# mlvlab/RPO

Hardware: AMD Instinct MI355X
Metric: images/sec (train step, ViT-B/16 K=24) (higher is better)
Workload: dtype bf16

## Files before the change

### rpo_amd/csrc/gemm_ws.hip

```cpp
#include "common.h"

#include <type_traits>

namespace {

struct WsParams {
  const char* A; int64_t lda;
  const char* Wp;
  char* C; int64_t ldc;
  int M, N, K;
  int tiles_m, tiles_n, split_k; int64_t split_stride;
  const float* bias;
  const float* resid; int64_t ldr;
  char* aux; int64_t ldaux; int aux_row0; int aux_mode;
  char* out2; int64_t ldout2; float* stats_out;
  const float* stats_in; const float* ln_colsum; float ln_eps; int ln_group;
  const char* pf_ptr; int64_t pf_bytes;
};

template <int N> __device__ __forceinline__ void ws_wait_vmcnt() {
  asm volatile("s_waitcnt vmcnt(%0)" ::"n"(N) : "memory");
}

__device__ __forceinline__ void ws_lds_barrier() { asm volatile("s_waitcnt lgkmcnt(0)\n\ts_barrier" ::: "memory"); }

template <int MT_, int NT_>
struct WsCfg {
  static constexpr int MT = MT_, NT = NT_, SLOTS = 2, THREADS = 256;
  static constexpr int BM = MT * 32, BN = NT * 32;
  static constexpr int SLOT_BYTES = BM * 128;
  static constexpr int WAVE_RING = SLOTS * SLOT_BYTES;
  static constexpr int RING_BYTES = 4 * WAVE_RING;
  static constexpr int FROW = BN * 4 + 16;
  static constexpr int PART_BYTES = 32 * FROW;
  static constexpr int STAGE_BYTES = 2 * 4 * PART_BYTES;
  static constexpr int STATS_BYTES = BM * 8;
  static constexpr int SMEM = (RING_BYTES > STAGE_BYTES ? RING_BYTES : STAGE_BYTES) + STATS_BYTES;
  static constexpr int DA = MT * 4;
  static constexpr int DW = NT * 4;
};

__device__ __forceinline__ float ws_row8_sum(float v) {
  v += __int_as_float(__builtin_amdgcn_update_dpp(0, __float_as_int(v), 0xB1, 0xf, 0xf, false));
  v += __int_as_float(__builtin_amdgcn_update_dpp(0, __float_as_int(v), 0x4E, 0xf, 0xf, false));
  v += __int_as_float(__builtin_amdgcn_update_dpp(0, __float_as_int(v), 0x141, 0xf, 0xf, false));
  return v;
}

__device__ __forceinline__ float2 ws_ln_finish(float mu_sum, float m2_sum, float sq_sum, int G, int K, float eps) {
  const float mu = mu_sum / (float)G;
  const float between = fmaxf(fmaf(-(float)G * mu, mu, sq_sum), 0.f);
  const float m2 = fmaf((float)(K / G), between, m2_sum);
  return make_float2(mu, rsqrtf(m2 / (float)K + eps));
}

template <typename T, typename TOut, int EPI, typename CF>
__global__ __launch_bounds__(256, 1) void gemm_ws_kernel(const WsParams p) {
  extern __shared__ __attribute__((aligned(128))) char smem[];
  constexpr int MT = CF::MT, NT = CF::NT;
  typedef const __attribute__((address_space(1))) void* gptr_t;
  typedef __attribute__((address_space(3))) void* lptr_t;
  const int tid = threadIdx.x;
  const int lane = tid & 63;
  const int wave = __builtin_amdgcn_readfirstlane(tid >> 6);
  const int half = lane >> 5, l31 = lane & 31;
  RPO_STAMP(0); RPO_STAMP_RT(62);

  int tile_m, tile_n, ksl;
  {
    const int nwg = gridDim.x, bid = blockIdx.x;
    const int qd = nwg >> 3, rm = nwg & 7, xcd = bid & 7;
    const int wg = (xcd < rm ? xcd * (qd + 1) : rm * (qd + 1) + (xcd - rm) * qd) + (bid >> 3);
    tile_m = wg % p.tiles_m;
    const int rest = wg / p.tiles_m;
    tile_n = rest % p.tiles_n;
    ksl = rest / p.tiles_n;
  }
  const int m0 = tile_m * CF::BM, n0 = tile_n * CF::BN;
  const int nch_all = p.K >> 6;
  const int wc0 = (int)(((int64_t)nch_all * ksl) / p.split_k), wc1 = (int)(((int64_t)nch_all * (ksl + 1)) / p.split_k);
  const int nwc = wc1 - wc0;
  const int c_lo = wc0 + (nwc * wave) / 4, c_hi = wc0 + (nwc * (wave + 1)) / 4;
  const int nc = c_hi - c_lo;

  uint32_t aoff[CF::DA];
  const int arow = lane >> 3;
  const uint32_t apark = (uint32_t)(arow * 128 + (((lane & 7) ^ ((arow >> 1) & 7)) << 4));
#pragma unroll
  for (int j = 0; j < CF::DA; ++j)
    aoff[j] = (uint32_t)min(m0 + 8 * j + arow, p.M - 1) * (uint32_t)(p.lda * 2) + (lane & 7) * 16;
  char* const ring = smem + wave * CF::WAVE_RING;
  const int KS = p.K >> 4;
  const char* wb[NT];
#pragma unroll
  for (int tn = 0; tn < NT; ++tn) {
    const int nb = min(n0 / 32 + tn, p.N / 32 - 1);
    wb[tn] = p.Wp + ((int64_t)nb * KS * 64 + lane) * 16;
  }
  const int sw = (l31 >> 1) & 7;
  uint32_t frag_off[4];
#pragma unroll
  for (int s = 0; s < 4; ++s) frag_off[s] = l31 * 128 + (((2 * s + half) ^ sw) << 4);

  f32x16_t acc[NT][MT];
#pragma unroll
  for (int a = 0; a < NT; ++a)
#pragma unroll
    for (int b = 0; b < MT; ++b)
#pragma unroll
      for (int r = 0; r < 16; ++r) acc[a][b][r] = 0.0f;

  constexpr bool IS_LN = EPI == RPO_EPI_LN_BIAS || EPI == RPO_EPI_LN_BIAS_QGELU;
  constexpr bool IS_QG = EPI == RPO_EPI_BIAS_QGELU || EPI == RPO_EPI_LN_BIAS_QGELU;
  constexpr bool HAS_BIAS = EPI == RPO_EPI_BIAS || EPI == RPO_EPI_BIAS_QGELU || EPI == RPO_EPI_BIAS_RESID || IS_LN;
  float2* const row_stats = reinterpret_cast<float2*>(smem + CF::SMEM - CF::STATS_BYTES);
  float2 lnp[IS_LN ? 16 : 1];
  const int G = IS_LN ? p.K / p.ln_group : 1;
  if constexpr (IS_LN) {
    if (tid < CF::BM) {
      const float2* ps = reinterpret_cast<const float2*>(p.stats_in) + (int64_t)min(m0 + tid, p.M - 1) * G;
#pragma unroll
      for (int g = 0; g < 16; ++g) lnp[g] = ps[min(g, G - 1)];
    }
  }
  const int row8 = lane >> 3, c8 = lane & 7;
  constexpr bool PRE_F32 = EPI == RPO_EPI_BIAS_RESID;
  constexpr bool PRE_AUX = EPI == RPO_EPI_QGELU_BWD;
  typedef __attribute__((ext_vector_type(4))) uint32_t u32x4_t;
  typedef __attribute__((ext_vector_type(2))) uint32_t u32x2_t;
  u32x4_t pre[(PRE_F32 || PRE_AUX) ? MT : 1][(PRE_F32 || PRE_AUX) ? NT : 1];
  if constexpr (PRE_F32 || PRE_AUX) {
    const bool wide = PRE_F32 || !p.aux_mode;
    const char* base = PRE_F32 ? reinterpret_cast<const char*>(p.resid) : p.aux;
    const int64_t ld = PRE_F32 ? p.ldr : p.ldaux;
#pragma unroll
    for (int tm = 0; tm < MT; ++tm) {
      const int m = min(m0 + tm * 32 + 8 * wave + row8, p.M - 1);
#pragma unroll
      for (int j = 0; j < NT; ++j) {
        const int n = min(n0 + 32 * j + 4 * c8, p.N - 4);
        if (wide) {
          pre[tm][j] = *reinterpret_cast<const u32x4_t*>(base + ((int64_t)m * ld + n) * 4);
        } else {
          const u32x2_t u = *reinterpret_cast<const u32x2_t*>(base + ((int64_t)m * ld + n) * 2);
          pre[tm][j] = u32x4_t{u.x, u.y, 0u, 0u};
        }
      }
    }
  }
  float4 b4[NT], s4[NT];
#pragma unroll
  for (int j = 0; j < NT; ++j) {
    const int n = min(n0 + 32 * j + 4 * c8, p.N - 4);
    b4[j] = HAS_BIAS ? *reinterpret_cast<const float4*>(p.bias + n) : make_float4(0.f, 0.f, 0.f, 0.f);
    s4[j] = IS_LN ? *reinterpret_cast<const float4*>(p.ln_colsum + n) : make_float4(0.f, 0.f, 0.f, 0.f);
  }
  bf16x8_t areg[CF::DA];
  bf16x8_t w[NT][4];
  constexpr int PPS = CF::DA / 4;
#define WS_PROLOGUE(NEXT)                                                                                              \
  {                                                                                                                      \
    const char* src = p.A + (int64_t)c_lo * 128;                                                                         \
    _Pragma("unroll") for (int j = 0; j < CF::DA; ++j) areg[j] = *reinterpret_cast<const bf16x8_t*>(src + aoff[j]);      \
    _Pragma("unroll") for (int s = 0; s < 4; ++s)                                                                        \
      _Pragma("unroll") for (int tn = 0; tn < NT; ++tn)                                                                  \
        w[tn][s] = *reinterpret_cast<const bf16x8_t*>(wb[tn] + (int64_t)(c_lo * 4 + s) * 1024);                          \
    _Pragma("unroll") for (int j = 0; j < CF::DA; ++j)                                                                   \
      *reinterpret_cast<bf16x8_t*>(ring + ((apark ^ (uint32_t)(((4 * j) & 7) << 4)) + j * 1024)) = areg[j];              \
    if (NEXT) {                                                                                                          \
      _Pragma("unroll") for (int j = 0; j < CF::DA; ++j)                                                                 \
        areg[j] = *reinterpret_cast<const bf16x8_t*>(src + 128 + aoff[j]);                                               \
    }                                                                                                                    \
    __builtin_amdgcn_sched_barrier(0);                                                                                   \
    RPO_STAMP(2);                                                                                                        \
  }
#define WS_CHUNK(REFRESH, PARK, LOAD)                                                                                  \
  {                                                                                                                      \
    const char* sb = ring + (i & 1) * CF::SLOT_BYTES;                                                                    \
    char* so = ring + ((i + 1) & 1) * CF::SLOT_BYTES;                                                                    \
    const char* asrc = p.A + (int64_t)(c_lo + i + 2) * 128;                                                              \
    _Pragma("unroll") for (int s = 0; s < 4; ++s) {                                                                      \
      bf16x8_t xf[MT];                                                                                                   \
      _Pragma("unroll") for (int tm = 0; tm < MT; ++tm)                                                                  \
        xf[tm] = *reinterpret_cast<const bf16x8_t*>(sb + tm * 4096 + frag_off[s]);                                       \
      _Pragma("unroll") for (int tn = 0; tn < NT; ++tn)                                                                  \
        _Pragma("unroll") for (int tm = 0; tm < MT; ++tm) acc[tn][tm] = mfma16<T>(w[tn][s], xf[tm], acc[tn][tm]);        \
      if (REFRESH) {                                                                                                     \
        _Pragma("unroll") for (int tn = 0; tn < NT; ++tn)                                                                \
          w[tn][s] = *reinterpret_cast<const bf16x8_t*>(wb[tn] + (int64_t)((c_lo + i + 1) * 4 + s) * 1024);              \
      }                                                                                                                  \
      _Pragma("unroll") for (int jj = 0; jj < PPS; ++jj) {                                                               \
        const int j = s * PPS + jj;                                                                                      \
        if (PARK) *reinterpret_cast<bf16x8_t*>(so + ((apark ^ (uint32_t)(((4 * j) & 7) << 4)) + j * 1024)) = areg[j];    \
        if (LOAD) areg[j] = *reinterpret_cast<const bf16x8_t*>(asrc + aoff[j]);                                          \
      }                                                                                                                  \
      __builtin_amdgcn_sched_barrier(0);             \
    }                                                                                                                    \
    RPO_STAMP(3 + (i < 40 ? i : 40));                                                                                    \
  }
  RPO_STAMP(1);
  if (nc >= 3) {
    WS_PROLOGUE(true)
    int i = 0;
    for (; i + 2 < nc; ++i) WS_CHUNK(true, true, true)
    WS_CHUNK(true, true, false)
    ++i;
    WS_CHUNK(false, false, false)
  } else if (nc == 2) {
    WS_PROLOGUE(true)
    int i = 0;
    WS_CHUNK(true, true, false)
    ++i;
    WS_CHUNK(false, false, false)
  } else if (nc == 1) {
    WS_PROLOGUE(false)
    const int i = 0;
    WS_CHUNK(false, false, false)
  }
#undef WS_PROLOGUE
#undef WS_CHUNK
  if constexpr (PRE_F32 || PRE_AUX) {
#pragma unroll
    for (int tm = 0; tm < MT; ++tm)
#pragma unroll
      for (int j = 0; j < NT; ++j) asm volatile("" :: "v"(pre[tm][j]));
  }
#pragma unroll
  for (int j = 0; j < NT; ++j) {
    if constexpr (HAS_BIAS) asm volatile("" :: "v"(b4[j].x), "v"(b4[j].y), "v"(b4[j].z), "v"(b4[j].w));
    if constexpr (IS_LN) asm volatile("" :: "v"(s4[j].x), "v"(s4[j].y), "v"(s4[j].z), "v"(s4[j].w));
  }
  if constexpr (IS_LN) {
#pragma unroll
    for (int g = 0; g < 16; ++g) asm volatile("" :: "v"(lnp[g].x), "v"(lnp[g].y));
  }
  uint32_t pf_touch;
  {
    const bool has = p.pf_ptr != nullptr;
    const char* base = has ? p.pf_ptr : p.Wp;
    const int64_t lines = has ? max(p.pf_bytes >> 7, (int64_t)1) : 1;
    const int64_t stride = (int64_t)gridDim.x * CF::THREADS;
    const int64_t i0 = (int64_t)blockIdx.x * CF::THREADS + tid;
    const char* t0 = base + (min(i0, lines - 1) << 7);
    const char* t1 = base + (min(i0 + stride, lines - 1) << 7);
    const char* t2 = base + (min(i0 + 2 * stride, lines - 1) << 7);
    const char* t3 = base + (min(i0 + 3 * stride, lines - 1) << 7);
    asm volatile("global_load_dword %0, %1, off\n\tglobal_load_dword %0, %2, off\n\t"
                 "global_load_dword %0, %3, off\n\tglobal_load_dword %0, %4, off"
                 : "=&v"(pf_touch) : "v"(t0), "v"(t1), "v"(t2), "v"(t3) : "memory");
  }

  if constexpr (IS_LN) {
    if (tid < CF::BM) {
      float mu = 0.f, m2 = 0.f, sq = 0.f;
#pragma unroll
      for (int g = 0; g < 16; ++g) {
        const float mg = g < G ? lnp[g].x : 0.f;
        mu += mg; m2 += g < G ? lnp[g].y : 0.f; sq = fmaf(mg, mg, sq);
      }
      row_stats[tid] = ws_ln_finish(mu, m2, sq, G, p.K, p.ln_eps);
    }
  }
  RPO_STAMP(58);
  ws_lds_barrier();
  RPO_STAMP(59);
  TOut* const cbase = reinterpret_cast<TOut*>(p.C) + (int64_t)ksl * p.split_stride;
  auto park = [&](const int tm) {
    char* mine = smem + (tm & 1) * (4 * CF::PART_BYTES) + wave * CF::PART_BYTES;
#pragma unroll
    for (int tn = 0; tn < NT; ++tn)
#pragma unroll
      for (int g = 0; g < 4; ++g)
        *reinterpret_cast<float4*>(mine + l31 * CF::FROW + (tn * 32 + 8 * g + 4 * half) * 4) =
            make_float4(acc[tn][tm][4 * g], acc[tn][tm][4 * g + 1], acc[tn][tm][4 * g + 2], acc[tn][tm][4 * g + 3]);
  };
  park(0);
#pragma unroll
  for (int tm = 0; tm < MT; ++tm) {
    const char* buf = smem + (tm & 1) * (4 * CF::PART_BYTES);
    const int row = tm * 32 + 8 * wave + row8;
    const int m = m0 + row;
    ws_lds_barrier();
    if (tm + 1 < MT) park(tm + 1);
    float4 v[NT];
#pragma unroll
    for (int j = 0; j < NT; ++j) {
      const char* src = buf + (8 * wave + row8) * CF::FROW + (32 * j + 4 * c8) * 4;
      const float4 p0 = *reinterpret_cast<const float4*>(src), p1 = *reinterpret_cast<const float4*>(src + CF::PART_BYTES);
      const float4 p2 = *reinterpret_cast<const float4*>(src + 2 * CF::PART_BYTES);
      const float4 p3 = *reinterpret_cast<const float4*>(src + 3 * CF::PART_BYTES);
      v[j] = make_float4((p0.x + p1.x) + (p2.x + p3.x), (p0.y + p1.y) + (p2.y + p3.y),
                         (p0.z + p1.z) + (p2.z + p3.z), (p0.w + p1.w) + (p2.w + p3.w));
    }
    float2 st = make_float2(0.f, 1.f);
    if constexpr (IS_LN) st = row_stats[row];
    float sum64 = 0.f;
#pragma unroll
    for (int j = 0; j < NT; ++j) {
      const int n = n0 + 32 * j + 4 * c8;
      const bool ok = m < p.M && n < p.N;
      float4 x = v[j];
      if constexpr (IS_LN) {
        x.x = fmaf(st.y, x.x - st.x * s4[j].x, b4[j].x); x.y = fmaf(st.y, x.y - st.x * s4[j].y, b4[j].y);
        x.z = fmaf(st.y, x.z - st.x * s4[j].z, b4[j].z); x.w = fmaf(st.y, x.w - st.x * s4[j].w, b4[j].w);
      } else if constexpr (HAS_BIAS) {
        x.x += b4[j].x; x.y += b4[j].y; x.z += b4[j].z; x.w += b4[j].w;
      }
      if constexpr (IS_QG) {
        if (p.aux != nullptr && ok && m >= p.aux_row0) {
          const int64_t off = (int64_t)(m - p.aux_row0) * p.ldaux + n;
          if (p.aux_mode)
            *reinterpret_cast<uint2*>(p.aux + off * 2) =
                make_uint2(pack2<T>(quick_gelu_grad(x.x), quick_gelu_grad(x.y)), pack2<T>(quick_gelu_grad(x.z), quick_gelu_grad(x.w)));
          else
            *reinterpret_cast<float4*>(p.aux + off * 4) = x;
        }
        x = quick_gelu4(x);
      }
      if constexpr (EPI == RPO_EPI_BIAS_RESID) {
        x.x += __uint_as_float(pre[tm][j].x); x.y += __uint_as_float(pre[tm][j].y);
        x.z += __uint_as_float(pre[tm][j].z); x.w += __uint_as_float(pre[tm][j].w);
      }
      if constexpr (EPI == RPO_EPI_QGELU_BWD) {
        float4 gq;
        if (p.aux_mode) {
          const uint32_t u0 = pre[tm][j].x, u1 = pre[tm][j].y;
          gq = make_float4(unpack1<T>((uint16_t)(u0 & 0xffffu)), unpack1<T>((uint16_t)(u0 >> 16)),
                           unpack1<T>((uint16_t)(u1 & 0xffffu)), unpack1<T>((uint16_t)(u1 >> 16)));
        } else {
          gq = make_float4(quick_gelu_grad(__uint_as_float(pre[tm][j].x)), quick_gelu_grad(__uint_as_float(pre[tm][j].y)),
                           quick_gelu_grad(__uint_as_float(pre[tm][j].z)), quick_gelu_grad(__uint_as_float(pre[tm][j].w)));
        }
        x.x *= gq.x; x.y *= gq.y; x.z *= gq.z; x.w *= gq.w;
      }
      if (ok) ActIO<TOut>::st4(cbase + (int64_t)m * p.ldc + n, x.x, x.y, x.z, x.w);
      if constexpr (EPI == RPO_EPI_BIAS_RESID) {
        if (p.out2 != nullptr && ok) ActIO<T>::st4(reinterpret_cast<T*>(p.out2) + (int64_t)m * p.ldout2 + n, x.x, x.y, x.z, x.w);
        if (p.stats_out != nullptr) {
          sum64 += (x.x + x.y) + (x.z + x.w);
          v[j] = x;
          if (j & 1) {
            const float mean = ws_row8_sum(sum64) * (1.0f / 64.0f);
            float q = 0.f;
#pragma unroll
            for (int jj = j - 1; jj <= j; ++jj) {
              const float dx = v[jj].x - mean, dy = v[jj].y - mean, dz = v[jj].z - mean, dw = v[jj].w - mean;
              q += (dx * dx + dy * dy) + (dz * dz + dw * dw);
            }
            q = ws_row8_sum(q);
            if (ok && c8 == 0) reinterpret_cast<float2*>(p.stats_out)[(int64_t)m * (p.N / 64) + ((n0 + 32 * j) >> 6)] = make_float2(mean, q);
            sum64 = 0.f;
          }
        }
      }
    }
  }
#ifdef RPO_TIMELINE
  asm volatile("s_waitcnt vmcnt(0)" ::: "memory");
#endif
  RPO_STAMP(61); RPO_STAMP_RT(63);
  asm volatile("" :: "v"(pf_touch));
}

__global__ void ws_pack_kernel(const char* W, int64_t ldw, char* Wp, int N, int K) {
  const int64_t pieces = (int64_t)N * K / 8;
  const int KS = K >> 4;
  for (int64_t i = (int64_t)blockIdx.x * blockDim.x + threadIdx.x; i < pieces; i += (int64_t)gridDim.x * blockDim.x) {
    const int l = (int)(i & 63);
    const int64_t blk = i >> 6;
    const int ks = (int)(blk % KS);
    const int nb = (int)(blk / KS);
    const int row = nb * 32 + (l & 31), k0 = ks * 16 + (l >> 5) * 8;
    *reinterpret_cast<uint4*>(Wp + i * 16) = *reinterpret_cast<const uint4*>(W + ((int64_t)row * ldw + k0) * 2);
  }
}

struct WsPlan { int mt, nt; };

static bool ws_geometry_ok(int mt, int nt) { return (mt == 1 && nt == 1) || (mt == 1 && nt == 2) || (mt == 2 && nt == 2) || (mt == 3 && nt == 3); }
static WsPlan ws_choose(int M, int N, int K, int split_k, int epilogue, bool wants_stats, int forced) {
  if (forced > 0) {
    const WsPlan f{forced / 100, (forced / 10) % 10};
    return ws_geometry_ok(f.mt, f.nt) ? f : WsPlan{0, 0};
  }
  static const WsPlan cand[] = {{3, 3}, {2, 2}, {1, 2}, {1, 1}};
  const int cus = rpo_cu_count();
  WsPlan best{0, 0};
  double best_cost = 0;
  for (const WsPlan& c : cand) {
    if (wants_stats && c.nt != 2) continue;
    const int64_t wgs = (int64_t)((M + 32 * c.mt - 1) / (32 * c.mt)) * ((N + 32 * c.nt - 1) / (32 * c.nt)) * split_k;
    const int64_t per_cu = (wgs + cus - 1) / cus;
    const double bytes = (double)(c.mt + c.nt) * 32 * (K / split_k) * 2;
    const double cost = per_cu * (bytes + 60e3 + 12e3 * c.mt * c.nt);
    if (best.mt == 0 || cost < best_cost) { best = c; best_cost = cost; }
  }
  return best;
}

template <typename T, typename TOut, int EPI, typename CF>
int ws_launch_t(WsParams& p, hipStream_t s) {
  static rpo_lds_mask_t lds_ok{0};
  auto kern = gemm_ws_kernel<T, TOut, EPI, CF>;
  if (int rc = rpo_allow_lds(reinterpret_cast<const void*>(kern), CF::SMEM, &lds_ok)) return rc;
  p.tiles_m = (p.M + CF::BM - 1) / CF::BM;
  p.tiles_n = (p.N + CF::BN - 1) / CF::BN;
  hipLaunchKernelGGL(kern, dim3(p.tiles_m * p.tiles_n * p.split_k), dim3(CF::THREADS), CF::SMEM, s, p);
  return rpo_launch_status();
}

template <typename T, typename TOut, int EPI>
int ws_launch(WsParams& p, const WsPlan& q, hipStream_t s, bool plan_only) {
  if (plan_only) return ws_geometry_ok(q.mt, q.nt) ? 100 * q.mt + 10 * q.nt : RPO_E_SHAPE;
  if (q.mt == 3 && q.nt == 3) return ws_launch_t<T, TOut, EPI, WsCfg<3, 3>>(p, s);
  if (q.mt == 2 && q.nt == 2) return ws_launch_t<T, TOut, EPI, WsCfg<2, 2>>(p, s);
  if (q.mt == 1 && q.nt == 2) return ws_launch_t<T, TOut, EPI, WsCfg<1, 2>>(p, s);
  if (q.mt == 1 && q.nt == 1) return ws_launch_t<T, TOut, EPI, WsCfg<1, 1>>(p, s);
  return RPO_E_SHAPE;
}

template <typename T>
int ws_dispatch(int epi, bool out16, WsParams& p, const WsPlan& q, hipStream_t s, bool plan_only) {
  switch (epi) {
    case RPO_EPI_NONE:
      return out16 ? ws_launch<T, T, RPO_EPI_NONE>(p, q, s, plan_only) : ws_launch<T, float, RPO_EPI_NONE>(p, q, s, plan_only);
    case RPO_EPI_QGELU_BWD:
      return out16 ? ws_launch<T, T, RPO_EPI_QGELU_BWD>(p, q, s, plan_only) : RPO_E_DTYPE;
    case RPO_EPI_BIAS:
      return out16 ? ws_launch<T, T, RPO_EPI_BIAS>(p, q, s, plan_only) : RPO_E_DTYPE;
    case RPO_EPI_BIAS_QGELU:
      return out16 ? ws_launch<T, T, RPO_EPI_BIAS_QGELU>(p, q, s, plan_only) : RPO_E_DTYPE;
    case RPO_EPI_LN_BIAS:
      return out16 ? ws_launch<T, T, RPO_EPI_LN_BIAS>(p, q, s, plan_only) : RPO_E_DTYPE;
    case RPO_EPI_LN_BIAS_QGELU:
      return out16 ? ws_launch<T, T, RPO_EPI_LN_BIAS_QGELU>(p, q, s, plan_only) : RPO_E_DTYPE;
    case RPO_EPI_BIAS_RESID:
      return out16 ? RPO_E_DTYPE : ws_launch<T, float, RPO_EPI_BIAS_RESID>(p, q, s, plan_only);
    default: return RPO_E_SHAPE;
  }
}

static int ws_prepare(const rpo_gemm_args* a, WsParams& p, WsPlan& q) {
  if (a == nullptr || a->M <= 0 || a->N <= 0 || a->K <= 0) return RPO_E_BADARG;
  const bool in16 = a->in_dtype == RPO_BF16 || a->in_dtype == RPO_F16;
  const bool out16 = a->out_dtype == RPO_BF16 || a->out_dtype == RPO_F16;
  if (!in16 || (out16 && a->out_dtype != a->in_dtype) || (!out16 && a->out_dtype != RPO_F32)) return RPO_E_DTYPE;
  if (a->K % 64 != 0 || a->N % 32 != 0) return RPO_E_SHAPE;
  if ((int64_t)a->M * a->lda * 2 >= (1ll << 32)) return RPO_E_SHAPE;
  const int epi = a->epilogue;
  const bool is_ln = epi == RPO_EPI_LN_BIAS || epi == RPO_EPI_LN_BIAS_QGELU;
  const bool needs_bias = epi == RPO_EPI_BIAS || epi == RPO_EPI_BIAS_QGELU || epi == RPO_EPI_BIAS_RESID || is_ln;
  if (epi == RPO_EPI_PATCH || epi < 0 || epi > RPO_EPI_LN_BIAS_QGELU) return RPO_E_SHAPE;
  if (a->skip_row0 >= 0 || a->resid_hi != nullptr || a->resid_lo != nullptr || a->out_lo != nullptr || a->c_row0 != 0 ||
      a->seg_rows0 != 0 || a->seg_rows1 != 0) return RPO_E_SHAPE;
  const int split = a->split_k <= 1 ? 1 : a->split_k;
  if (split > 1 && (epi != RPO_EPI_NONE || out16 || split > a->K / 64 || a->split_stride % 4 != 0)) return RPO_E_SHAPE;
  if (needs_bias && (a->bias == nullptr || !aligned16(a->bias))) return RPO_E_BADARG;
  if (is_ln) {
    const int g = a->ln_group == 0 ? 64 : a->ln_group;
    if (a->ln_stats == nullptr || a->ln_colsum == nullptr || !aligned16(a->ln_colsum) || !(a->ln_eps > 0.0f) ||
        reinterpret_cast<uintptr_t>(a->ln_stats) % 8 != 0) return RPO_E_BADARG;
    if ((g != 64 && g != 96) || a->K % g != 0 || a->K / g > 16) return RPO_E_SHAPE;
  }
  if (!is_ln && epi != RPO_EPI_BIAS_RESID && (a->ln_stats != nullptr || a->out2 != nullptr)) return RPO_E_BADARG;
  const bool wants_stats = epi == RPO_EPI_BIAS_RESID && a->ln_stats != nullptr;
  if (epi == RPO_EPI_BIAS_RESID) {
    if (a->resid == nullptr || !aligned16(a->resid) || a->ldr % 4 != 0) return RPO_E_BADARG;
    if (a->out2 != nullptr && (reinterpret_cast<uintptr_t>(a->out2) % 8 != 0 || (a->ldout2 * 2) % 8 != 0)) return RPO_E_ALIGN;
    if (wants_stats && (a->N % 64 != 0 || (a->ln_group != 0 && a->ln_group != 64) ||
                        reinterpret_cast<uintptr_t>(a->ln_stats) % 8 != 0)) return RPO_E_SHAPE;
  }
  if (epi == RPO_EPI_QGELU_BWD && a->aux == nullptr) return RPO_E_BADARG;
  if (a->aux != nullptr && (epi == RPO_EPI_QGELU_BWD || epi == RPO_EPI_BIAS_QGELU || epi == RPO_EPI_LN_BIAS_QGELU)) {
    if (!aligned16(a->aux) || a->ldaux % 4 != 0) return RPO_E_ALIGN;
    if (a->aux_dtype != RPO_F32 && a->aux_dtype != a->in_dtype) return RPO_E_DTYPE;
  }
  const int osz = out16 ? 2 : 4;
  if (!aligned16(a->A) || (a->lda * 2) % 16 != 0 || !aligned16(a->W)) return RPO_E_ALIGN;
  if ((reinterpret_cast<uintptr_t>(a->C) % (4 * osz)) != 0 || (a->ldc * osz) % (4 * osz) != 0) return RPO_E_ALIGN;
  q = ws_choose(a->M, a->N, a->K, split, epi, wants_stats, a->tile_config);
  if (q.mt == 0 || (wants_stats && q.nt != 2)) return RPO_E_SHAPE;
  p = WsParams{};
  p.A = static_cast<const char*>(a->A); p.lda = a->lda;
  p.Wp = static_cast<const char*>(a->W);
  p.C = static_cast<char*>(a->C); p.ldc = a->ldc;
  p.M = a->M; p.N = a->N; p.K = a->K;
  p.split_k = split; p.split_stride = a->split_stride;
  p.bias = a->bias; p.resid = a->resid; p.ldr = a->ldr;
  p.aux = static_cast<char*>(a->aux); p.ldaux = a->ldaux; p.aux_row0 = a->aux_row0;
  p.aux_mode = (a->aux != nullptr && a->aux_dtype != RPO_F32) ? 1 : 0;
  p.out2 = static_cast<char*>(a->out2); p.ldout2 = a->ldout2;
  p.stats_out = wants_stats ? a->ln_stats : nullptr;
  p.stats_in = is_ln ? a->ln_stats : nullptr;
  p.ln_colsum = a->ln_colsum; p.ln_eps = a->ln_eps; p.ln_group = a->ln_group == 0 ? 64 : a->ln_group;
  p.pf_ptr = static_cast<const char*>(a->prefetch);
  p.pf_bytes = a->prefetch == nullptr ? 0 : a->prefetch_bytes;
  if (p.pf_bytes < 0 || (p.pf_ptr != nullptr && reinterpret_cast<uintptr_t>(p.pf_ptr) % 4 != 0)) return RPO_E_BADARG;
  return 0;
}

}

extern "C" int rpo_gemm_ws_pack(const void* W, int64_t ldw, void* Wp, int N, int K, int dtype, void* stream) {
  if (W == nullptr || Wp == nullptr || N <= 0 || K <= 0) return RPO_E_BADARG;
  if (dtype != RPO_BF16 && dtype != RPO_F16) return RPO_E_DTYPE;
  if (N % 32 != 0 || K % 64 != 0) return RPO_E_SHAPE;
  if (!aligned16(W) || !aligned16(Wp) || (ldw * 2) % 16 != 0) return RPO_E_ALIGN;
  const int64_t pieces = (int64_t)N * K / 8;
  const int blocks = (int)((pieces + 255) / 256 < 4096 ? (pieces + 255) / 256 : 4096);
  hipLaunchKernelGGL(ws_pack_kernel, dim3(blocks), dim3(256), 0, static_cast<hipStream_t>(stream),
                     static_cast<const char*>(W), ldw, static_cast<char*>(Wp), N, K);
  return rpo_launch_status();
}

extern "C" int rpo_gemm_ws_ok(const rpo_gemm_args* a) {
  WsParams p;
  WsPlan q;
  if (a == nullptr) return 0;
  rpo_gemm_args b = *a;
  static const uintptr_t dummy = 4096;
  auto fill = [](const void*& ptr) { if (ptr == nullptr) ptr = reinterpret_cast<const void*>(dummy); };
  fill(b.A); fill(b.W);
  if (b.C == nullptr) b.C = reinterpret_cast<void*>(dummy);
  const int epi = b.epilogue;
  const bool is_ln = epi == RPO_EPI_LN_BIAS || epi == RPO_EPI_LN_BIAS_QGELU;
  if (epi == RPO_EPI_BIAS || epi == RPO_EPI_BIAS_QGELU || epi == RPO_EPI_BIAS_RESID || is_ln)
    if (b.bias == nullptr) b.bias = reinterpret_cast<const float*>(dummy);
  if (epi == RPO_EPI_BIAS_RESID && b.resid == nullptr) { b.resid = reinterpret_cast<const float*>(dummy); if (b.ldr == 0) b.ldr = b.N; }
  if (epi == RPO_EPI_QGELU_BWD && b.aux == nullptr) { b.aux = reinterpret_cast<void*>(dummy); if (b.ldaux == 0) b.ldaux = b.N; }
  if (is_ln) {
    if (b.ln_stats == nullptr) b.ln_stats = reinterpret_cast<float*>(dummy);
    if (b.ln_colsum == nullptr) b.ln_colsum = reinterpret_cast<const float*>(dummy);
    if (!(b.ln_eps > 0.0f)) b.ln_eps = 1e-5f;
  }
  return ws_prepare(&b, p, q) == 0 ? 1 : 0;
}

static int ws_run(const rpo_gemm_args* a, hipStream_t s, bool plan_only) {
  WsParams p;
  WsPlan q;
  if (a == nullptr || a->A == nullptr || a->W == nullptr || a->C == nullptr) return RPO_E_BADARG;
  if (int rc = ws_prepare(a, p, q)) return rc;
  const bool out16 = a->out_dtype != RPO_F32;
  if (a->in_dtype == RPO_F16) return ws_dispatch<f16_t>(a->epilogue, out16, p, q, s, plan_only);
  return ws_dispatch<bf16_t>(a->epilogue, out16, p, q, s, plan_only);
}

extern "C" int rpo_gemm_ws(const rpo_gemm_args* a, void* stream) {
  return ws_run(a, static_cast<hipStream_t>(stream), false);
}

extern "C" int rpo_gemm_ws_plan(const rpo_gemm_args* a) {
  return ws_run(a, nullptr, true);
}
```

Baseline: 11370.

## Precompute tile-map reciprocals, overlap epilogue operand loads, batch epilogue reduction rounds

Replaces the per-block integer divisions used to map workgroup IDs to tiles and K-chunks with reciprocal multiplies that are precomputed on the host. The epilogue operand loads (LN stats, residual/aux, bias, colsum) now issue inside the prologue, right after the first A/W loads, so their latency overlaps the main loop. The epilogue reduction now parks several M-blocks per LDS round (two for MT=3), which cuts the number of barriers. In exchange, more registers stay live across the main loop, which could lower occupancy or cause spills, and there is added shape validation for the reciprocal math.

```diff
diff --git a/rpo_amd/csrc/gemm_ws.hip b/rpo_amd/csrc/gemm_ws.hip
--- a/rpo_amd/csrc/gemm_ws.hip
+++ b/rpo_amd/csrc/gemm_ws.hip
@@ -1,4 +1,5 @@
 #include "common.h"
+#include "ws_map.h"
 
 #include <type_traits>
 
@@ -9,12 +10,12 @@
   const char* Wp;
   char* C; int64_t ldc;
   int M, N, K;
-  int tiles_m, tiles_n, split_k; int64_t split_stride;
+  WsMap map; int split_k; int64_t split_stride;
   const float* bias;
   const float* resid; int64_t ldr;
   char* aux; int64_t ldaux; int aux_row0; int aux_mode;
   char* out2; int64_t ldout2; float* stats_out;
-  const float* stats_in; const float* ln_colsum; float ln_eps; int ln_group;
+  const float* stats_in; const float* ln_colsum; float ln_eps; int ln_ngroups;
   const char* pf_ptr; int64_t pf_bytes;
 };
 
@@ -33,7 +34,8 @@
   static constexpr int RING_BYTES = 4 * WAVE_RING;
   static constexpr int FROW = BN * 4 + 16;
   static constexpr int PART_BYTES = 32 * FROW;
-  static constexpr int STAGE_BYTES = 2 * 4 * PART_BYTES;
+  static constexpr int ROUND_BLOCKS = MT == 3 ? 2 : MT;
+  static constexpr int STAGE_BYTES = ROUND_BLOCKS * 4 * PART_BYTES;
   static constexpr int STATS_BYTES = BM * 8;
   static constexpr int SMEM = (RING_BYTES > STAGE_BYTES ? RING_BYTES : STAGE_BYTES) + STATS_BYTES;
   static constexpr int DA = MT * 4;
@@ -71,16 +73,12 @@
     const int nwg = gridDim.x, bid = blockIdx.x;
     const int qd = nwg >> 3, rm = nwg & 7, xcd = bid & 7;
     const int wg = (xcd < rm ? xcd * (qd + 1) : rm * (qd + 1) + (xcd - rm) * qd) + (bid >> 3);
-    tile_m = wg % p.tiles_m;
-    const int rest = wg / p.tiles_m;
-    tile_n = rest % p.tiles_n;
-    ksl = rest / p.tiles_n;
+    ws_map_tile(p.map, (uint32_t)wg, tile_m, tile_n, ksl);
   }
   const int m0 = tile_m * CF::BM, n0 = tile_n * CF::BN;
-  const int nch_all = p.K >> 6;
-  const int wc0 = (int)(((int64_t)nch_all * ksl) / p.split_k), wc1 = (int)(((int64_t)nch_all * (ksl + 1)) / p.split_k);
+  const int wc0 = ws_map_chunk0(p.map, ksl), wc1 = ws_map_chunk0(p.map, ksl + 1);
   const int nwc = wc1 - wc0;
-  const int c_lo = wc0 + (nwc * wave) / 4, c_hi = wc0 + (nwc * (wave + 1)) / 4;
+  const int c_lo = wc0 + ((nwc * wave) >> 2), c_hi = wc0 + ((nwc * (wave + 1)) >> 2);
   const int nc = c_hi - c_lo;
 
   uint32_t aoff[CF::DA];
@@ -94,7 +92,7 @@
   const char* wb[NT];
 #pragma unroll
   for (int tn = 0; tn < NT; ++tn) {
-    const int nb = min(n0 / 32 + tn, p.N / 32 - 1);
+    const int nb = min(tile_n * NT + tn, (p.N >> 5) - 1);
     wb[tn] = p.Wp + ((int64_t)nb * KS * 64 + lane) * 16;
   }
   const int sw = (l31 >> 1) & 7;
@@ -114,57 +112,61 @@
   constexpr bool IS_QG = EPI == RPO_EPI_BIAS_QGELU || EPI == RPO_EPI_LN_BIAS_QGELU;
   constexpr bool HAS_BIAS = EPI == RPO_EPI_BIAS || EPI == RPO_EPI_BIAS_QGELU || EPI == RPO_EPI_BIAS_RESID || IS_LN;
   float2* const row_stats = reinterpret_cast<float2*>(smem + CF::SMEM - CF::STATS_BYTES);
+  const int row8 = lane >> 3, c8 = lane & 7;
   float2 lnp[IS_LN ? 16 : 1];
-  const int G = IS_LN ? p.K / p.ln_group : 1;
-  if constexpr (IS_LN) {
-    if (tid < CF::BM) {
-      const float2* ps = reinterpret_cast<const float2*>(p.stats_in) + (int64_t)min(m0 + tid, p.M - 1) * G;
-#pragma unroll
-      for (int g = 0; g < 16; ++g) lnp[g] = ps[min(g, G - 1)];
-    }
-  }
-  const int row8 = lane >> 3, c8 = lane & 7;
+  const int G = IS_LN ? p.ln_ngroups : 1;
   constexpr bool PRE_F32 = EPI == RPO_EPI_BIAS_RESID;
   constexpr bool PRE_AUX = EPI == RPO_EPI_QGELU_BWD;
   typedef __attribute__((ext_vector_type(4))) uint32_t u32x4_t;
   typedef __attribute__((ext_vector_type(2))) uint32_t u32x2_t;
   u32x4_t pre[(PRE_F32 || PRE_AUX) ? MT : 1][(PRE_F32 || PRE_AUX) ? NT : 1];
-  if constexpr (PRE_F32 || PRE_AUX) {
-    const bool wide = PRE_F32 || !p.aux_mode;
-    const char* base = PRE_F32 ? reinterpret_cast<const char*>(p.resid) : p.aux;
-    const int64_t ld = PRE_F32 ? p.ldr : p.ldaux;
-#pragma unroll
-    for (int tm = 0; tm < MT; ++tm) {
-      const int m = min(m0 + tm * 32 + 8 * wave + row8, p.M - 1);
-#pragma unroll
-      for (int j = 0; j < NT; ++j) {
-        const int n = min(n0 + 32 * j + 4 * c8, p.N - 4);
-        if (wide) {
-          pre[tm][j] = *reinterpret_cast<const u32x4_t*>(base + ((int64_t)m * ld + n) * 4);
-        } else {
-          const u32x2_t u = *reinterpret_cast<const u32x2_t*>(base + ((int64_t)m * ld + n) * 2);
-          pre[tm][j] = u32x4_t{u.x, u.y, 0u, 0u};
+  float4 b4[NT], s4[NT];
+  auto request_tail_operands = [&]() __attribute__((always_inline)) {
+    if constexpr (IS_LN) {
+      const float2* ps = reinterpret_cast<const float2*>(p.stats_in) + (int64_t)min(m0 + min(tid, CF::BM - 1), p.M - 1) * G;
+#pragma unroll
+      for (int g = 0; g < 16; ++g) lnp[g] = ps[min(g, G - 1)];
+    }
+    if constexpr (PRE_F32 || PRE_AUX) {
+      const bool wide = PRE_F32 || !p.aux_mode;
+      const char* base = PRE_F32 ? reinterpret_cast<const char*>(p.resid) : p.aux;
+      const int64_t ld = PRE_F32 ? p.ldr : p.ldaux;
+#pragma unroll
+      for (int tm = 0; tm < MT; ++tm) {
+        const int m = min(m0 + tm * 32 + 8 * wave + row8, p.M - 1);
+#pragma unroll
+        for (int j = 0; j < NT; ++j) {
+          const int n = min(n0 + 32 * j + 4 * c8, p.N - 4);
+          if (wide) {
+            pre[tm][j] = *reinterpret_cast<const u32x4_t*>(base + ((int64_t)m * ld + n) * 4);
+          } else {
+            const u32x2_t u = *reinterpret_cast<const u32x2_t*>(base + ((int64_t)m * ld + n) * 2);
+            pre[tm][j] = u32x4_t{u.x, u.y, 0u, 0u};
+          }
         }
       }
     }
-  }
-  float4 b4[NT], s4[NT];
-#pragma unroll
-  for (int j = 0; j < NT; ++j) {
-    const int n = min(n0 + 32 * j + 4 * c8, p.N - 4);
-    b4[j] = HAS_BIAS ? *reinterpret_cast<const float4*>(p.bias + n) : make_float4(0.f, 0.f, 0.f, 0.f);
-    s4[j] = IS_LN ? *reinterpret_cast<const float4*>(p.ln_colsum + n) : make_float4(0.f, 0.f, 0.f, 0.f);
-  }
+#pragma unroll
+    for (int j = 0; j < NT; ++j) {
+      const int n = min(n0 + 32 * j + 4 * c8, p.N - 4);
+      b4[j] = HAS_BIAS ? *reinterpret_cast<const float4*>(p.bias + n) : make_float4(0.f, 0.f, 0.f, 0.f);
+      s4[j] = IS_LN ? *reinterpret_cast<const float4*>(p.ln_colsum + n) : make_float4(0.f, 0.f, 0.f, 0.f);
+    }
+  };
   bf16x8_t areg[CF::DA];
   bf16x8_t w[NT][4];
   constexpr int PPS = CF::DA / 4;
 #define WS_PROLOGUE(NEXT)                                                                                              \
   {                                                                                                                      \
     const char* src = p.A + (int64_t)c_lo * 128;                                                                         \
+    RPO_STAMP(1);                                                                                                        \
     _Pragma("unroll") for (int j = 0; j < CF::DA; ++j) areg[j] = *reinterpret_cast<const bf16x8_t*>(src + aoff[j]);      \
     _Pragma("unroll") for (int s = 0; s < 4; ++s)                                                                        \
       _Pragma("unroll") for (int tn = 0; tn < NT; ++tn)                                                                  \
         w[tn][s] = *reinterpret_cast<const bf16x8_t*>(wb[tn] + (int64_t)(c_lo * 4 + s) * 1024);                          \
+    __builtin_amdgcn_sched_barrier(0);                                                                                   \
+    request_tail_operands();                                                                                             \
+    __builtin_amdgcn_sched_barrier(0);                                                                                   \
     _Pragma("unroll") for (int j = 0; j < CF::DA; ++j)                                                                   \
       *reinterpret_cast<bf16x8_t*>(ring + ((apark ^ (uint32_t)(((4 * j) & 7) << 4)) + j * 1024)) = areg[j];              \
     if (NEXT) {                                                                                                          \
@@ -198,7 +200,6 @@
     }                                                                                                                    \
     RPO_STAMP(3 + (i < 40 ? i : 40));                                                                                    \
   }
-  RPO_STAMP(1);
   if (nc >= 3) {
     WS_PROLOGUE(true)
     int i = 0;
@@ -216,6 +217,8 @@
     WS_PROLOGUE(false)
     const int i = 0;
     WS_CHUNK(false, false, false)
+  } else {
+    request_tail_operands();
   }
 #undef WS_PROLOGUE
 #undef WS_CHUNK
@@ -265,91 +268,100 @@
   ws_lds_barrier();
   RPO_STAMP(59);
   TOut* const cbase = reinterpret_cast<TOut*>(p.C) + (int64_t)ksl * p.split_stride;
-  auto park = [&](const int tm) {
-    char* mine = smem + (tm & 1) * (4 * CF::PART_BYTES) + wave * CF::PART_BYTES;
-#pragma unroll
-    for (int tn = 0; tn < NT; ++tn)
-#pragma unroll
-      for (int g = 0; g < 4; ++g)
-        *reinterpret_cast<float4*>(mine + l31 * CF::FROW + (tn * 32 + 8 * g + 4 * half) * 4) =
-            make_float4(acc[tn][tm][4 * g], acc[tn][tm][4 * g + 1], acc[tn][tm][4 * g + 2], acc[tn][tm][4 * g + 3]);
-  };
-  park(0);
-#pragma unroll
-  for (int tm = 0; tm < MT; ++tm) {
-    const char* buf = smem + (tm & 1) * (4 * CF::PART_BYTES);
-    const int row = tm * 32 + 8 * wave + row8;
-    const int m = m0 + row;
+  constexpr int RB = CF::ROUND_BLOCKS;
+#pragma unroll
+  for (int t0 = 0; t0 < MT; t0 += RB) {
+    if (t0 > 0) ws_lds_barrier();
+#pragma unroll
+    for (int tm = t0; tm < MT && tm < t0 + RB; ++tm) {
+      char* mine = smem + ((tm - t0) * 4 + wave) * CF::PART_BYTES;
+#pragma unroll
+      for (int tn = 0; tn < NT; ++tn)
+#pragma unroll
+        for (int g = 0; g < 4; ++g)
+          *reinterpret_cast<float4*>(mine + l31 * CF::FROW + (tn * 32 + 8 * g + 4 * half) * 4) =
+              make_float4(acc[tn][tm][4 * g], acc[tn][tm][4 * g + 1], acc[tn][tm][4 * g + 2], acc[tn][tm][4 * g + 3]);
+    }
     ws_lds_barrier();
-    if (tm + 1 < MT) park(tm + 1);
-    float4 v[NT];
-#pragma unroll
-    for (int j = 0; j < NT; ++j) {
-      const char* src = buf + (8 * wave + row8) * CF::FROW + (32 * j + 4 * c8) * 4;
-      const float4 p0 = *reinterpret_cast<const float4*>(src), p1 = *reinterpret_cast<const float4*>(src + CF::PART_BYTES);
-      const float4 p2 = *reinterpret_cast<const float4*>(src + 2 * CF::PART_BYTES);
-      const float4 p3 = *reinterpret_cast<const float4*>(src + 3 * CF::PART_BYTES);
-      v[j] = make_float4((p0.x + p1.x) + (p2.x + p3.x), (p0.y + p1.y) + (p2.y + p3.y),
-                         (p0.z + p1.z) + (p2.z + p3.z), (p0.w + p1.w) + (p2.w + p3.w));
-    }
-    float2 st = make_float2(0.f, 1.f);
-    if constexpr (IS_LN) st = row_stats[row];
-    float sum64 = 0.f;
-#pragma unroll
-    for (int j = 0; j < NT; ++j) {
-      const int n = n0 + 32 * j + 4 * c8;
-      const bool ok = m < p.M && n < p.N;
-      float4 x = v[j];
-      if constexpr (IS_LN) {
-        x.x = fmaf(st.y, x.x - st.x * s4[j].x, b4[j].x); x.y = fmaf(st.y, x.y - st.x * s4[j].y, b4[j].y);
-        x.z = fmaf(st.y, x.z - st.x * s4[j].z, b4[j].z); x.w = fmaf(st.y, x.w - st.x * s4[j].w, b4[j].w);
-      } else if constexpr (HAS_BIAS) {
-        x.x += b4[j].x; x.y += b4[j].y; x.z += b4[j].z; x.w += b4[j].w;
+    float4 vr[RB][NT];
+    float2 str[RB];
+#pragma unroll
+    for (int tm = t0; tm < MT && tm < t0 + RB; ++tm) {
+      const char* buf = smem + (tm - t0) * (4 * CF::PART_BYTES);
+#pragma unroll
+      for (int j = 0; j < NT; ++j) {
+        const char* src = buf + (8 * wave + row8) * CF::FROW + (32 * j + 4 * c8) * 4;
+        const float4 p0 = *reinterpret_cast<const float4*>(src), p1 = *reinterpret_cast<const float4*>(src + CF::PART_BYTES);
+        const float4 p2 = *reinterpret_cast<const float4*>(src + 2 * CF::PART_BYTES);
+        const float4 p3 = *reinterpret_cast<const float4*>(src + 3 * CF::PART_BYTES);
+        vr[tm - t0][j] = make_float4((p0.x + p1.x) + (p2.x + p3.x), (p0.y + p1.y) + (p2.y + p3.y),
+                                     (p0.z + p1.z) + (p2.z + p3.z), (p0.w + p1.w) + (p2.w + p3.w));
       }
-      if constexpr (IS_QG) {
-        if (p.aux != nullptr && ok && m >= p.aux_row0) {
-          const int64_t off = (int64_t)(m - p.aux_row0) * p.ldaux + n;
-          if (p.aux_mode)
-            *reinterpret_cast<uint2*>(p.aux + off * 2) =
-                make_uint2(pack2<T>(quick_gelu_grad(x.x), quick_gelu_grad(x.y)), pack2<T>(quick_gelu_grad(x.z), quick_gelu_grad(x.w)));
-          else
-            *reinterpret_cast<float4*>(p.aux + off * 4) = x;
+      str[tm - t0] = make_float2(0.f, 1.f);
+      if constexpr (IS_LN) str[tm - t0] = row_stats[tm * 32 + 8 * wave + row8];
+    }
+#pragma unroll
+    for (int tm = t0; tm < MT && tm < t0 + RB; ++tm) {
+      const int m = m0 + tm * 32 + 8 * wave + row8;
+      float4 (&v)[NT] = vr[tm - t0];
+      const float2 st = str[tm - t0];
+      float sum64 = 0.f;
+#pragma unroll
+      for (int j = 0; j < NT; ++j) {
+        const int n = n0 + 32 * j + 4 * c8;
+        const bool ok = m < p.M && n < p.N;
+        float4 x = v[j];
+        if constexpr (IS_LN) {
+          x.x = fmaf(st.y, x.x - st.x * s4[j].x, b4[j].x); x.y = fmaf(st.y, x.y - st.x * s4[j].y, b4[j].y);
+          x.z = fmaf(st.y, x.z - st.x * s4[j].z, b4[j].z); x.w = fmaf(st.y, x.w - st.x * s4[j].w, b4[j].w);
+        } else if constexpr (HAS_BIAS) {
+          x.x += b4[j].x; x.y += b4[j].y; x.z += b4[j].z; x.w += b4[j].w;
         }
-        x = quick_gelu4(x);
-      }
-      if constexpr (EPI == RPO_EPI_BIAS_RESID) {
-        x.x += __uint_as_float(pre[tm][j].x); x.y += __uint_as_float(pre[tm][j].y);
-        x.z += __uint_as_float(pre[tm][j].z); x.w += __uint_as_float(pre[tm][j].w);
-      }
-      if constexpr (EPI == RPO_EPI_QGELU_BWD) {
-        float4 gq;
-        if (p.aux_mode) {
-          const uint32_t u0 = pre[tm][j].x, u1 = pre[tm][j].y;
-          gq = make_float4(unpack1<T>((uint16_t)(u0 & 0xffffu)), unpack1<T>((uint16_t)(u0 >> 16)),
-                           unpack1<T>((uint16_t)(u1 & 0xffffu)), unpack1<T>((uint16_t)(u1 >> 16)));
-        } else {
-          gq = make_float4(quick_gelu_grad(__uint_as_float(pre[tm][j].x)), quick_gelu_grad(__uint_as_float(pre[tm][j].y)),
-                           quick_gelu_grad(__uint_as_float(pre[tm][j].z)), quick_gelu_grad(__uint_as_float(pre[tm][j].w)));
+        if constexpr (IS_QG) {
+          if (p.aux != nullptr && ok && m >= p.aux_row0) {
+            const int64_t off = (int64_t)(m - p.aux_row0) * p.ldaux + n;
+            if (p.aux_mode)
+              *reinterpret_cast<uint2*>(p.aux + off * 2) =
+                  make_uint2(pack2<T>(quick_gelu_grad(x.x), quick_gelu_grad(x.y)), pack2<T>(quick_gelu_grad(x.z), quick_gelu_grad(x.w)));
+            else
+              *reinterpret_cast<float4*>(p.aux + off * 4) = x;
+          }
+          x = quick_gelu4(x);
         }
-        x.x *= gq.x; x.y *= gq.y; x.z *= gq.z; x.w *= gq.w;
-      }
-      if (ok) ActIO<TOut>::st4(cbase + (int64_t)m * p.ldc + n, x.x, x.y, x.z, x.w);
-      if constexpr (EPI == RPO_EPI_BIAS_RESID) {
-        if (p.out2 != nullptr && ok) ActIO<T>::st4(reinterpret_cast<T*>(p.out2) + (int64_t)m * p.ldout2 + n, x.x, x.y, x.z, x.w);
-        if (p.stats_out != nullptr) {
-          sum64 += (x.x + x.y) + (x.z + x.w);
-          v[j] = x;
-          if (j & 1) {
-            const float mean = ws_row8_sum(sum64) * (1.0f / 64.0f);
-            float q = 0.f;
-#pragma unroll
-            for (int jj = j - 1; jj <= j; ++jj) {
-              const float dx = v[jj].x - mean, dy = v[jj].y - mean, dz = v[jj].z - mean, dw = v[jj].w - mean;
-              q += (dx * dx + dy * dy) + (dz * dz + dw * dw);
+        if constexpr (EPI == RPO_EPI_BIAS_RESID) {
+          x.x += __uint_as_float(pre[tm][j].x); x.y += __uint_as_float(pre[tm][j].y);
+          x.z += __uint_as_float(pre[tm][j].z); x.w += __uint_as_float(pre[tm][j].w);
+        }
+        if constexpr (EPI == RPO_EPI_QGELU_BWD) {
+          float4 gq;
+          if (p.aux_mode) {
+            const uint32_t u0 = pre[tm][j].x, u1 = pre[tm][j].y;
+            gq = make_float4(unpack1<T>((uint16_t)(u0 & 0xffffu)), unpack1<T>((uint16_t)(u0 >> 16)),
+                             unpack1<T>((uint16_t)(u1 & 0xffffu)), unpack1<T>((uint16_t)(u1 >> 16)));
+          } else {
+            gq = make_float4(quick_gelu_grad(__uint_as_float(pre[tm][j].x)), quick_gelu_grad(__uint_as_float(pre[tm][j].y)),
+                             quick_gelu_grad(__uint_as_float(pre[tm][j].z)), quick_gelu_grad(__uint_as_float(pre[tm][j].w)));
+          }
+          x.x *= gq.x; x.y *= gq.y; x.z *= gq.z; x.w *= gq.w;
+        }
+        if (ok) ActIO<TOut>::st4(cbase + (int64_t)m * p.ldc + n, x.x, x.y, x.z, x.w);
+        if constexpr (EPI == RPO_EPI_BIAS_RESID) {
+          if (p.out2 != nullptr && ok) ActIO<T>::st4(reinterpret_cast<T*>(p.out2) + (int64_t)m * p.ldout2 + n, x.x, x.y, x.z, x.w);
+          if (p.stats_out != nullptr) {
+            sum64 += (x.x + x.y) + (x.z + x.w);
+            v[j] = x;
+            if (j & 1) {
+              const float mean = ws_row8_sum(sum64) * (1.0f / 64.0f);
+              float q = 0.f;
+#pragma unroll
+              for (int jj = j - 1; jj <= j; ++jj) {
+                const float dx = v[jj].x - mean, dy = v[jj].y - mean, dz = v[jj].z - mean, dw = v[jj].w - mean;
+                q += (dx * dx + dy * dy) + (dz * dz + dw * dw);
+              }
+              q = ws_row8_sum(q);
+              if (ok && c8 == 0) reinterpret_cast<float2*>(p.stats_out)[(int64_t)m * (p.N / 64) + ((n0 + 32 * j) >> 6)] = make_float2(mean, q);
+              sum64 = 0.f;
             }
-            q = ws_row8_sum(q);
-            if (ok && c8 == 0) reinterpret_cast<float2*>(p.stats_out)[(int64_t)m * (p.N / 64) + ((n0 + 32 * j) >> 6)] = make_float2(mean, q);
-            sum64 = 0.f;
           }
         }
       }
@@ -403,9 +415,7 @@
   static rpo_lds_mask_t lds_ok{0};
   auto kern = gemm_ws_kernel<T, TOut, EPI, CF>;
   if (int rc = rpo_allow_lds(reinterpret_cast<const void*>(kern), CF::SMEM, &lds_ok)) return rc;
-  p.tiles_m = (p.M + CF::BM - 1) / CF::BM;
-  p.tiles_n = (p.N + CF::BN - 1) / CF::BN;
-  hipLaunchKernelGGL(kern, dim3(p.tiles_m * p.tiles_n * p.split_k), dim3(CF::THREADS), CF::SMEM, s, p);
+  hipLaunchKernelGGL(kern, dim3(p.map.tiles_m * p.map.tiles_n * p.split_k), dim3(CF::THREADS), CF::SMEM, s, p);
   return rpo_launch_status();
 }
 
@@ -480,7 +490,10 @@
   if ((reinterpret_cast<uintptr_t>(a->C) % (4 * osz)) != 0 || (a->ldc * osz) % (4 * osz) != 0) return RPO_E_ALIGN;
   q = ws_choose(a->M, a->N, a->K, split, epi, wants_stats, a->tile_config);
   if (q.mt == 0 || (wants_stats && q.nt != 2)) return RPO_E_SHAPE;
+  const int tiles_m = (a->M + 32 * q.mt - 1) / (32 * q.mt), tiles_n = (a->N + 32 * q.nt - 1) / (32 * q.nt);
+  if (!ws_map_ok(tiles_m, tiles_n, split)) return RPO_E_SHAPE;
   p = WsParams{};
+  p.map = ws_map_make(tiles_m, tiles_n, split, a->K / 64);
   p.A = static_cast<const char*>(a->A); p.lda = a->lda;
   p.Wp = static_cast<const char*>(a->W);
   p.C = static_cast<char*>(a->C); p.ldc = a->ldc;
@@ -492,7 +505,7 @@
   p.out2 = static_cast<char*>(a->out2); p.ldout2 = a->ldout2;
   p.stats_out = wants_stats ? a->ln_stats : nullptr;
   p.stats_in = is_ln ? a->ln_stats : nullptr;
-  p.ln_colsum = a->ln_colsum; p.ln_eps = a->ln_eps; p.ln_group = a->ln_group == 0 ? 64 : a->ln_group;
+  p.ln_colsum = a->ln_colsum; p.ln_eps = a->ln_eps; p.ln_ngroups = a->K / (a->ln_group == 0 ? 64 : a->ln_group);
   p.pf_ptr = static_cast<const char*>(a->prefetch);
   p.pf_bytes = a->prefetch == nullptr ? 0 : a->prefetch_bytes;
   if (p.pf_bytes < 0 || (p.pf_ptr != nullptr && reinterpret_cast<uintptr_t>(p.pf_ptr) % 4 != 0)) return RPO_E_BADARG;
diff --git a/rpo_amd/csrc/ws_map.h b/rpo_amd/csrc/ws_map.h
--- /dev/null
+++ b/rpo_amd/csrc/ws_map.h
@@ -0,0 +1,45 @@
+#pragma once
+
+#include <cstdint>
+
+#if defined(__HIP__) || defined(__HIPCC__) || defined(__CUDACC__)
+#define WS_MAP_HD __host__ __device__ __forceinline__
+#else
+#define WS_MAP_HD inline
+#endif
+
+struct WsMap {
+  uint32_t tiles_m, tiles_n;
+  uint32_t rcp_tm, rcp_tn, rcp_split;
+  uint32_t k_base, k_rem;
+};
+
+WS_MAP_HD uint32_t ws_rcp(uint32_t d) { return (uint32_t)(0x80000000u / d); }
+WS_MAP_HD uint32_t ws_rcp_div(uint32_t n, uint32_t rcp) { return (uint32_t)(((uint64_t)(2u * n + 1u) * rcp) >> 32); }
+
+WS_MAP_HD bool ws_map_ok(int64_t tiles_m, int64_t tiles_n, int64_t split_k) {
+  const int64_t nwg = tiles_m * tiles_n * split_k;
+  const int64_t nmax = nwg > split_k * split_k ? nwg : split_k * split_k;
+  const int64_t dmax = tiles_m > tiles_n ? (tiles_m > split_k ? tiles_m : split_k) : (tiles_n > split_k ? tiles_n : split_k);
+  return tiles_m > 0 && tiles_n > 0 && split_k > 0 && nwg < (1ll << 31) && (2 * nmax + 1) * dmax < (1ll << 31);
+}
+
+WS_MAP_HD WsMap ws_map_make(int tiles_m, int tiles_n, int split_k, int nch_all) {
+  WsMap m;
+  m.tiles_m = (uint32_t)tiles_m; m.tiles_n = (uint32_t)tiles_n;
+  m.rcp_tm = ws_rcp(m.tiles_m); m.rcp_tn = ws_rcp(m.tiles_n); m.rcp_split = ws_rcp((uint32_t)split_k);
+  m.k_base = (uint32_t)(nch_all / split_k); m.k_rem = (uint32_t)(nch_all % split_k);
+  return m;
+}
+
+WS_MAP_HD void ws_map_tile(const WsMap& m, uint32_t wg, int& tile_m, int& tile_n, int& ksl) {
+  const uint32_t rest = ws_rcp_div(wg, m.rcp_tm);
+  const uint32_t ks = ws_rcp_div(rest, m.rcp_tn);
+  tile_m = (int)(wg - rest * m.tiles_m);
+  tile_n = (int)(rest - ks * m.tiles_n);
+  ksl = (int)ks;
+}
+
+WS_MAP_HD int ws_map_chunk0(const WsMap& m, int ksl) {
+  return (int)(m.k_base * (uint32_t)ksl + ws_rcp_div(m.k_rem * (uint32_t)ksl, m.rcp_split));
+}
```

New measurement: 11420 (median of 6 runs). No clear change (+0.5%).
